# 21cmfast/21cmFAST

Hardware: AMD Instinct MI355X
Metric: IonizeBox cells/sec (512^3 HII_DIM, 40 filter radii) (higher is better)
Workload: dtype f32; 1 GPU; ComputeIonizedBox single-z, HII_DIM=512, 40 filter steps, G=2 (delta tophat + n_ion exp-MFP), first snapshot, device-resident inputs; hii_dim=512, n_radii=40, filtered_grids=2, parallelism=single GPU, fft=native

## Files before the change

### 21cmfast_amd/csrc/hip/c21hip.h

```cpp
#ifndef C21HIP_H
#define C21HIP_H

#include <stddef.h>

#include "ws_slots.h"

#ifdef __cplusplus
extern "C" {
#endif

int c21hip_device_count(void);
int c21hip_current_device(void);
int c21hip_use_device(int device);
int c21hip_is_device_ptr(const void *p);
void *c21hip_ws(int slot, size_t bytes);
__attribute__((visibility("hidden"))) const void *c21_stage_in(int slot, const void *p, size_t bytes, void *stream, int *status);
void *c21hip_ws_peek(int slot, size_t *bytes);
int c21hip_ws_adopt(int slot, void *ptr, size_t bytes);
void *c21hip_raw_alloc(size_t bytes);
void *c21hip_vmm_chunk(size_t phys_bytes, size_t map_bytes, void **va_out);
void c21hip_vmm_chunk_free(void *chunk);
int c21hip_ws_adopt_vmm(int slot, void *chunk, size_t bytes);
void c21hip_raw_free(void *p);
size_t c21hip_free_bytes(void);
// ... 146 lines not shown
int c21hip_split_fold_multi(const float *hi_split, float *const lo_split[4], const int ops[4], int n_out, int nx,
                            int ny, int nz, int f, double box_len, double box_len_z, float tophat_R, void *stream);
int c21hip_lpt2_source(const float *const diag[3], const float *const off[3], float *out, size_t n,
                       float norm, void *stream);
int c21hip_copy_filter_split(const float *src_split, float *dst_split, int nx, int ny, int nz,
                             double box_len, double box_len_z, int filter_type, float R,
                             float R_param, int apply, void *stream);
int c21hip_split_z_c2r(const float *split_work, float *real_out, long out_zstride, int nx, int ny,
                       int nz, void *stream);
int c21hip_split_z_ionise_stars(const float *delta_work, const float *stars_work,
                                unsigned char *first_cross, double *partials, double *sum_out,
                                int nx, int ny, int nz, int r_index, double rhocrit_omb,
                                double ion_eff, int mass_dep_zeta, double f_limit, void *stream);
int c21hip_z_ionise_partials(int nx, int ny, int nz);
int c21hip_batched_means(const double *partials, long stride, int n_partials, int first, int step,
                         int count, double ntot, int mass_dep_zeta, double f_limit, double *sums,
                         double *means, void *stream);
int c21hip_split_z_ionise_stars_xe(const float *delta_work, const float *stars_work,
                                   const float *xe_work, unsigned char *first_cross,
                                   double *partials, double *sum_out, int nx, int ny, int nz,
                                   int r_index, double rhocrit_omb, double ion_eff,
                                   int mass_dep_zeta, double f_limit, void *stream);
int c21hip_z_ionise_xe_supported(int nx, int ny, int nz);
int c21hip_split_filter_xy_shared(const float *src, float *work, int filter_type, int nx, int ny,
                                  int nz, double box_len, double box_len_z, float R, int apply,
                                  int table_slot, void *stream);
int c21hip_bench_pass(int kind, int n, int filter_a, int filter_b, float R, float R_param_b,
                      double box_len, int reps, void *stream, float *ms_out);
int c21hip_reduce_sum(const double *partials, int n, double *out, void *stream);
int c21hip_reduce_op(const double *partials, int n, int op, double *stage, double *out,
                     void *stream);

int c21hip_pack_clip(const float *dense, float *padded, int nx, int ny, int nz, double factor,
                     double lo, double hi, void *stream);
int c21hip_unpack_scale(const float *padded, float *dense, int nx, int ny, int nz, float scale,
                        void *stream);
int c21hip_divide_inplace(float *buf, size_t n, float divisor, void *stream);
int c21hip_divide_inplace_f64(float *buf, size_t n, double divisor, void *stream);
int c21hip_fill(float *buf, size_t n, float value, void *stream);
int c21hip_add_scalar(float *buf, size_t n, float value, void *stream);
int c21hip_widen(const float *in, double *out, size_t n, void *stream);

int c21hip_copy_filter(const float *src_c, float *dst_c, int nx, int ny, int nz, double box_len,
                       double box_len_z, int filter_type, float R, float R_param, int apply,
                       void *stream);
int c21hip_copy_filter_star(const float *src_c, float *dst_c, int nx, int ny, int nz,
// ... 377 lines not shown
```

### 21cmfast_amd/csrc/hip/fft_native.hip

```cpp
#include <hip/hip_runtime.h>

#include <cmath>
#include <map>
#include <mutex>
#include <vector>

#include "c21hip.h"
#include "fcoll_device.h"
#include "ms_window.h"
#include "c21cm_abi.h"
#include "c21cm_grid.h"

#ifndef C21X_XPAIR_THREADS
#define C21X_XPAIR_THREADS 512
#endif
#ifndef C21X_FUSE512
#define C21X_FUSE512 1
#endif
#ifndef C21X_FUSE1024
#define C21X_FUSE1024 1
#endif
#ifndef C21X_F512_MERGE
#define C21X_F512_MERGE 1
#endif
// ... 1536 lines not shown
        } else {
            const float2 A = tile[k * ZROW + li], B = tile[(H - k) * ZROW + li];
            const float2 E = make_float2(0.5f * (A.x + B.x), 0.5f * (A.y - B.y));
            const float2 D = make_float2(0.5f * (A.x - B.x), 0.5f * (A.y + B.y));
            const float2 wD = cmul(D, twN[k]);
            tile[k * ZROW + li] = make_float2(E.x + wD.y, E.y - wD.x);
            tile[(H - k) * ZROW + li] = make_float2(E.x - wD.y, -E.y - wD.x);
        }
    }
    __syncthreads();
#pragma unroll
    for (int u = 0; u < NIN; u++) {
        const int f = threadIdx.x + kBlock * u;
        const int li = f / H, k = f % H;
        a.main[(l0 + li) * H + k] = tile[k * ZROW + li];
    }
}

struct ZFusedArgs {
    const float2 *d_main, *d_nyq;
    const float2 *s_main, *s_nyq;
    const float2 *x_main, *x_nyq;
    unsigned char *first_cross;
    double *partials;
    double rhocrit_omb, ion_eff, f_limit;
    int mass_dep_zeta, r_index;
    int ny, lb;
    int store_all;
    int reverse;
    int rc;
    const float *nrec;
    double rec0;
    int x_is_nrec;
    const float2 *n_main, *n_nyq;
    float *g12;
};

template <int NZ>
__global__ void __launch_bounds__(kBlock)
z_c2r_ionise_kernel(ZFusedArgs a, const float2 *__restrict__ twH_global,
                    const float2 *__restrict__ twN_global) {
    constexpr int H = NZ / 2, LZ = LZ_FUSED, ZROW = LZ + 1;
    constexpr int NOUT = ZGeom<NZ, LZ>::NOUT;
    extern __shared__ float4 lds_raw[];
    float2 *tile = reinterpret_cast<float2 *>(lds_raw);
    float2 *twH = tile + H * ZROW;
// ... 267 lines not shown

template <int NZ, int EPI = 0>
int launch_z_c2r(const ZPassArgs &a, long nlines, hipStream_t stream) {
    constexpr int H = NZ / 2;
    const float2 *twH = twiddles(H);
    const float2 *twN = twiddles(NZ);
    if (!twH || !twN) return C21CM_MEMORY_ALLOC_ERROR;
    const size_t lds = sizeof(float2) * ((size_t)H * (LZ_PLAIN + 1) + H + H / 2 + 1);
    static bool attr_done = false;
    if (!attr_done) {
        (void)hipFuncSetAttribute((const void *)z_c2r_kernel<NZ, EPI>,
                                  hipFuncAttributeMaxDynamicSharedMemorySize, (int)lds);
        attr_done = true;
    }
    hipLaunchKernelGGL((z_c2r_kernel<NZ, EPI>), dim3((unsigned)(nlines / LZ_PLAIN)), dim3(kBlock),
                       lds, stream, a, twH, twN);
    LAUNCH_CHECK();
    return 0;
}

constexpr int ZW_LINES = 16;
constexpr int zw_lines(int P) { return kBlock / P; }

template <int A, bool TS, int P = 16, bool RC = false>
__global__ void
#if C21X_ZW_OCC
__launch_bounds__(kBlock, (A == 16 && !TS) ? C21X_ZW_OCC : 1)
#else
__launch_bounds__((A == 16 && P == 16) ? C21X_ZW_BLOCK : kBlock, (TS && RC && A == 16 && P == 16) ? C21X_ZW_TSRC_OCC : 1)
#endif
zw_ionise_kernel(ZFusedArgs a, const float2 *__restrict__ twH_global,
                 const float2 *__restrict__ twN_global) {
    constexpr int ZBLK = (A == 16 && P == 16) ? C21X_ZW_BLOCK : kBlock;
    constexpr int H = P * A, NZ = 2 * H, ZWL = ZBLK / P;
    constexpr int LINE_LDS = A * (P + 1) + 4;
    static_assert(LINE_LDS % 2 == 0, "16-byte aligned line regions (mask rows)");
    __shared__ __attribute__((aligned(16))) float2 lines[ZWL * LINE_LDS];
    __shared__ float2 twH[H], twN[H];
    __shared__ double red[ZBLK / 64];
    for (int t = threadIdx.x; t < H; t += ZBLK) {
        twH[t] = twH_global[t];
        twN[t] = twN_global[t];
    }
    const int lane = threadIdx.x & 63, wave = threadIdx.x >> 6;
    const int g = lane / P, b = lane % P;
    const int lw = wave * (64 / P) + g;
    const unsigned blk = a.reverse ? gridDim.x - 1 - blockIdx.x : blockIdx.x;
    const long line = (long)blk * ZWL + lw;
    float2 *L = lines + lw * LINE_LDS;
    const float2 *dm = a.d_main + line * H, *sm = a.s_main + line * H;
    constexpr bool EARLY = (A == 16) && !C21X_ZW_LATE;
    float2 xd[A], xs[A];
#pragma unroll
    for (int q = 0; q < A; q++) xd[q] = dm[P * q + b];
    if (EARLY) {
#pragma unroll
        for (int q = 0; q < A; q++) xs[q] = sm[P * q + b];
    }
    const long lline = logical_line(line, a.ny, a.lb);
    const float dh = a.d_nyq[lline].x, sh = a.s_nyq[lline].x;
    unsigned char *mrow = a.first_cross + lline * NZ;
    constexpr bool MASK16 = EARLY && (C21X_ZW_MASK16 || (TS && RC && C21X_ZW_TSRC_LEAN));
    constexpr int MV = MASK16 ? A / 8 : 1;
    uint4 mreg[MV];
    uchar2 old[(EARLY && !MASK16) ? A : 1];
    if constexpr (MASK16) {
#pragma unroll
        for (int v = 0; v < MV; v++) mreg[v] = reinterpret_cast<const uint4 *>(mrow)[b * MV + v];
    } else if (EARLY) {
#pragma unroll
        for (int q = 0; q < A; q++)
            old[q] = reinterpret_cast<const uchar2 *>(mrow)[(b + P * (q / P)) + A * (q % P)];
    }
    constexpr bool STASH = TS && RC && A == 16 && P == 16 && C21X_ZW_TSRC_LEAN;
    constexpr int NRH = (RC && A == 16 && !STASH) ? A / 2 : 1;
    float2 nr_lo[NRH], nr_hi[NRH];
    __shared__ __attribute__((aligned(16))) float nstash[STASH ? ZWL * NZ : 4];
    uint4 nreg[STASH ? NZ / (4 * P) : 1];
    if constexpr (STASH) {
#pragma unroll
        for (int v = 0; v < NZ / (4 * P); v++) nreg[v] = make_uint4(0u, 0u, 0u, 0u);
        if (a.nrec) {
#pragma unroll
            for (int v = 0; v < NZ / (4 * P); v++)
                nreg[v] = reinterpret_cast<const uint4 *>(a.nrec + lline * NZ)[v * P + b];
        }
    } else if constexpr (RC && A == 16) {
        if (a.nrec) {
#pragma unroll
            for (int q = 0; q < NRH; q++)
                nr_lo[q] = reinterpret_cast<const float2 *>(a.nrec + lline * NZ)[(b + P * (q / P)) + A * (q % P)];
        }
// ... 39 lines not shown
        wave_fence();
        wave_c2r<A, P>(xx, xh, L, twH, twN, b);
    }

    if constexpr (RC && A == 16 && !STASH) {
        if (a.nrec) {
#pragma unroll
            for (int q = 0; q < NRH; q++) {
                const int qq = q + NRH;
                nr_hi[q] = reinterpret_cast<const float2 *>(a.nrec + lline * NZ)[(b + P * (qq / P)) + A * (qq % P)];
            }
        }
    }
    if constexpr (MASK16) {
        wave_fence();
#pragma unroll
        for (int v = 0; v < MV; v++) reinterpret_cast<uint4 *>(L)[b * MV + v] = mreg[v];
        wave_fence();
    }
    const double floor_lhs = a.f_limit * a.ion_eff;
    const bool floor_ionises = !TS && a.mass_dep_zeta && (floor_lhs > 1.);
    const float dmin = (float)(-1. + 1e-7);
    double acc = 0.;
#pragma unroll
    for (int q = 0; q < A; q++) {
        const int j = (b + P * (q / P)) + A * (q % P);
        const float s0 = fmaxf(xs[q].x, 0.f), s1 = fmaxf(xs[q].y, 0.f);
        acc += (double)s0;
        acc += (double)s1;
        double D0 = a.rhocrit_omb * (1. + (double)fmaxf(xd[q].x, dmin));
        double D1 = a.rhocrit_omb * (1. + (double)fmaxf(xd[q].y, dmin));
        bool f0 = false, f1 = false;
        if constexpr (TS) {
            const double n0 = 1. - (double)fminf(fmaxf(xx[q].x, 0.f), 0.999f);
            const double n1 = 1. - (double)fminf(fmaxf(xx[q].y, 0.f), 0.999f);
            f0 = a.mass_dep_zeta && floor_lhs > n0;
            f1 = a.mass_dep_zeta && floor_lhs > n1;
            D0 *= n0;
            D1 *= n1;
        }
        double opd0 = 1., opd1 = 1.;
        if constexpr (RC) {
            opd0 = 1. + (double)fmaxf(xd[q].x, dmin);
            opd1 = 1. + (double)fmaxf(xd[q].y, dmin);
            double r0 = a.rec0, r1 = a.rec0;
            if (a.nrec || (STASH && a.n_main)) {
                const float2 nr = STASH ? reinterpret_cast<const float2 *>(nstash + lw * NZ)[j]
                                  : (A == 16) ? (q < NRH ? nr_lo[(A == 16 && !STASH && q < NRH) ? q : 0]
                                                         : nr_hi[(A == 16 && !STASH && q >= NRH) ? q - NRH : 0])
                                              : reinterpret_cast<const float2 *>(a.nrec + lline * NZ)[j];
                r0 = (double)nr.x, r1 = (double)nr.y;
            }
            double n0 = 1., n1 = 1.;
            if constexpr (TS) {
                if (a.x_is_nrec) {
                    r0 = (double)fmaxf(xx[q].x, 0.f);
                    r1 = (double)fmaxf(xx[q].y, 0.f);
                } else {
                    n0 = 1. - (double)fminf(fmaxf(xx[q].x, 0.f), 0.999f);
                    n1 = 1. - (double)fminf(fmaxf(xx[q].y, 0.f), 0.999f);
                }
            }
            D0 = a.rhocrit_omb * ((opd0 + r0) * n0);
            D1 = a.rhocrit_omb * ((opd1 + r1) * n1);
            f0 = a.mass_dep_zeta && floor_lhs * opd0 > (opd0 + r0) * n0;
            f1 = a.mass_dep_zeta && floor_lhs * opd1 > (opd1 + r1) * n1;
        }
        const bool i0 = (!RC && floor_ionises) || f0 || ((double)s0 * a.ion_eff > D0);
        const bool i1 = (!RC && floor_ionises) || f1 || ((double)s1 * a.ion_eff > D1);
        uchar2 m = MASK16 ? reinterpret_cast<const uchar2 *>(L)[j]
                          : (EARLY ? old[(EARLY && !MASK16) ? q : 0] : reinterpret_cast<const uchar2 *>(mrow)[j]);
        const bool n0 = i0 && m.x == 0, n1 = i1 && m.y == 0;
        if (n0) m.x = (unsigned char)a.r_index;
        if (n1) m.y = (unsigned char)a.r_index;
        if constexpr (MASK16) {
            if (n0 || n1) reinterpret_cast<uchar2 *>(L)[j] = m;
        } else if (n0 || n1 || a.store_all)
            reinterpret_cast<uchar2 *>(mrow)[j] = m;
        if constexpr (RC) {
            float *grow = a.g12 + lline * NZ + 2 * j;
            if (n0 && a.rc != 2) grow[0] = fmaxf(xd[q].x, dmin);
            if (n1 && a.rc != 2) grow[1] = fmaxf(xd[q].y, dmin);
        }
#if C21X_ZW_TSRC_FENCE
        if constexpr (TS && RC) __builtin_amdgcn_sched_barrier(0);
#endif
    }
    if constexpr (MASK16) {
        wave_fence();
#pragma unroll
        for (int v = 0; v < MV; v++) {
            const uint4 n = reinterpret_cast<const uint4 *>(L)[b * MV + v], o = mreg[v];
            if (a.store_all || n.x != o.x || n.y != o.y || n.z != o.z || n.w != o.w)
                reinterpret_cast<uint4 *>(mrow)[b * MV + v] = n;
        }
    }
#pragma unroll
    for (int off = 32; off > 0; off >>= 1) acc += __shfl_down(acc, off, 64);
    if (lane == 0) red[wave] = acc;
    __syncthreads();
    if (threadIdx.x == 0) {
        double sum = 0.;
#pragma unroll
        for (int w = 0; w < ZBLK / 64; w++) sum += red[w];
        a.partials[blk] = sum;
    }
}

template <int A, int EPI, int P = 16>
__global__ void __launch_bounds__(kBlock)
zw_c2r_kernel(ZPassArgs a, const float2 *__restrict__ twH_global,
              const float2 *__restrict__ twN_global) {
    constexpr int H = P * A, NZ = 2 * H, ZWL = zw_lines(P);
    constexpr int LINE_LDS = A * (P + 1) + 4;
    static_assert(LINE_LDS % 2 == 0, "16-byte aligned line regions (EPI 7)");
    __shared__ __attribute__((aligned(16))) float2 lines[ZWL * LINE_LDS];
    __shared__ float2 twH[H], twN[H];
    for (int t = threadIdx.x; t < H; t += kBlock) {
        twH[t] = twH_global[t];
// ... 597 lines not shown

template <int NZ>
int launch_z_fused(const ZFusedArgs &a, long nlines, hipStream_t stream) {
    constexpr int H = NZ / 2;
    const float2 *twH = twiddles(H);
    const float2 *twN = twiddles(NZ);
    if (!twH || !twN) return C21CM_MEMORY_ALLOC_ERROR;
    const size_t lds = sizeof(float2) * ((size_t)H * (LZ_FUSED + 1) + H + H / 2 + 1);
    static bool attr_done = false;
    if (!attr_done) {
        (void)hipFuncSetAttribute((const void *)z_c2r_ionise_kernel<NZ>,
                                  hipFuncAttributeMaxDynamicSharedMemorySize, (int)lds);
        attr_done = true;
    }
    hipLaunchKernelGGL((z_c2r_ionise_kernel<NZ>), dim3((unsigned)(nlines / LZ_FUSED)), dim3(kBlock), lds,
                       stream, a, twH, twN);
    LAUNCH_CHECK();
    return 0;
}

int dispatch_z_fused(int nz, const ZFusedArgs &a, long nlines, hipStream_t stream, int *n_partials) {
    KTimeScope kt(2, stream);
    *n_partials = (int)(nlines / LZ_FUSED);
    if (a.rc && (zw3_selected(nz, nlines) || !zw_lines_of(nz, nlines))) {
        c21hip_set_error("fused pass Z with recombinations needs the 16-lane wave kernel (z-lines of 256 / 512 points)");
        return C21CM_VALUE_ERROR;
    }
    if (zw3_selected(nz, nlines)) {
        const float2 *twH = twiddles(nz / 2);
        const float2 *twN = twiddles(nz);
        if (!twH || !twN) return C21CM_MEMORY_ALLOC_ERROR;
        *n_partials = (int)(nlines / (kBlock / 64));
        const dim3 grid((unsigned)(nlines / (kBlock / 64)));
        if (a.x_main)
            hipLaunchKernelGGL(zw3_ionise_kernel<true>, grid, dim3(kBlock), 0, stream, a, twH, twN);
        else
            hipLaunchKernelGGL(zw3_ionise_kernel<false>, grid, dim3(kBlock), 0, stream, a, twH, twN);
        LAUNCH_CHECK();
        return 0;
    }
    if (int zwl = zw_lines_of(nz, nlines)) {
        const float2 *twH = twiddles(nz / 2);
        const float2 *twN = twiddles(nz);
        if (!twH || !twN) return C21CM_MEMORY_ALLOC_ERROR;
        const int zblk = (nz == 512) ? C21X_ZW_BLOCK : kBlock;
        if (nz == 512) zwl = zblk / 16;
// ... 8 lines not shown
                hipLaunchKernelGGL((zw_ionise_kernel<16, true, 8, true>), grid, dim3(zblk), 0, stream, a, twH, twN);
            else if (nz == 512)
                hipLaunchKernelGGL((zw_ionise_kernel<16, true, 16, true>), grid, dim3(zblk), 0, stream, a, twH, twN);
            else {
                c21hip_set_error("fused pass Z with recombinations and an x_e grid: 256- / 512-point z-lines only");
                return C21CM_VALUE_ERROR;
            }
        } else if (a.rc) {
            if (nz == 256)
                ZW_FUSED_RC(16, 8);
            else if (nz == 512)
                ZW_FUSED_RC(16, 16);
            else
                ZW_FUSED_RC(32, 16);
        } else if (a.x_main) {
            if (nz == 256)
                ZW_FUSED(16, true, 8);
            else if (nz == 512)
                ZW_FUSED(16, true, 16);
            else
                ZW_FUSED(32, true, 16);
        } else if (nz == 256)
            ZW_FUSED(16, false, 8);
        else if (nz == 512)
            ZW_FUSED(16, false, 16);
        else
            ZW_FUSED(32, false, 16);
#undef ZW_FUSED
#undef ZW_FUSED_RC
        LAUNCH_CHECK();
        return 0;
    }
    if (a.x_main) {
        c21hip_set_error("fused pass Z with an x_e grid needs 256-, 512- or 1024-point z-lines");
        return C21CM_VALUE_ERROR;
    }
    switch (nz) {
        case 64: return launch_z_fused<64>(a, nlines, stream);
        case 128: return launch_z_fused<128>(a, nlines, stream);
        case 192: return launch_z_fused<192>(a, nlines, stream);
        case 256: return launch_z_fused<256>(a, nlines, stream);
        case 384: return launch_z_fused<384>(a, nlines, stream);
        case 512: return launch_z_fused<512>(a, nlines, stream);
        case 768: return launch_z_fused<768>(a, nlines, stream);
        case 1024: return launch_z_fused<1024>(a, nlines, stream);
        case 1536: return launch_z_fused<1536>(a, nlines, stream);
// ... 1194 lines not shown
    return c21hip_reduce_sum(partials, (int)(nlines / LZ_PLAIN), sum_out, stream);
}

extern "C" int c21hip_split_filter_c2r(const float *split_src, float *split_work, float *real_out,
                                       long out_zstride, int nx, int ny, int nz, double box_len,
                                       double box_len_z, int filter_type, float R, float R_param,
                                       int apply, void *stream) {
    int st = c21hip_split_filter_xy(split_src, split_work, nx, ny, nz, box_len, box_len_z,
                                    filter_type, R, R_param, apply, stream);
    if (st) return st;
    return c21hip_split_z_c2r(split_work, real_out, out_zstride, nx, ny, nz, stream);
}

extern "C" int c21hip_split_z_ionise_stars(const float *delta_work, const float *stars_work,
                                           unsigned char *first_cross, double *partials,
                                           double *sum_out, int nx, int ny, int nz, int r_index,
                                           double rhocrit_omb, double ion_eff, int mass_dep_zeta,
                                           double f_limit, void *stream) {
    return c21hip_split_z_ionise_stars_xe(delta_work, stars_work, NULL, first_cross, partials,
                                          sum_out, nx, ny, nz, r_index, rhocrit_omb, ion_eff,
                                          mass_dep_zeta, f_limit, stream);
}

extern "C" int c21hip_split_z_ionise_stars_xe(const float *delta_work, const float *stars_work,
                                              const float *xe_work, unsigned char *first_cross,
                                              double *partials, double *sum_out, int nx, int ny,
                                              int nz, int r_index, double rhocrit_omb,
                                              double ion_eff, int mass_dep_zeta, double f_limit,
                                              void *stream) {
    const long nlines = (long)nx * ny;
    ZFusedArgs a{};
    a.ny = ny;
    a.lb = split_xb_log2(nx);
    a.d_main = reinterpret_cast<const float2 *>(delta_work);
    a.d_nyq = a.d_main + nlines * (nz / 2);
    a.s_main = reinterpret_cast<const float2 *>(stars_work);
    a.s_nyq = a.s_main + nlines * (nz / 2);
    if (xe_work) {
        a.x_main = reinterpret_cast<const float2 *>(xe_work);
        a.x_nyq = a.x_main + nlines * (nz / 2);
    }
    a.first_cross = first_cross;
    a.partials = partials;
    a.rhocrit_omb = rhocrit_omb;
    a.ion_eff = ion_eff;
    a.f_limit = f_limit;
    a.mass_dep_zeta = mass_dep_zeta;
    a.r_index = r_index;
    static const int store_all = [] {
        const char *e = getenv("C21CM_MASK_STORE_ALL");
        return (e && e[0] == '1') ? 1 : 0;
    }();
    a.store_all = store_all;
    static const int reverse = [] {
        const char *e = getenv("C21CM_ZREV");
        return (e && e[0] == '0') ? 0 : 1;
    }();
    a.reverse = reverse;
    int n_partials = 0;
    int st = dispatch_z_fused(nz, a, nlines, (hipStream_t)stream, &n_partials);
    if (st) return st;
    if (!sum_out) return 0;
    return c21hip_reduce_sum(partials, n_partials, sum_out, stream);
}

extern "C" int c21hip_split_z_ionise_recomb_xe(const float *delta_work, const float *stars_work,
                                               const float *xe_work, const float *nrec, double rec0,
                                               float *g12, unsigned char *first_cross, double *partials,
                                               int nx, int ny, int nz, int r_index, double rhocrit_omb,
                                               double ion_eff, int mass_dep_zeta, double f_limit,
                                               void *stream);
extern "C" int c21hip_split_z_ionise_recomb(const float *delta_work, const float *stars_work,
                                            const float *nrec, double rec0, float *g12,
                                            unsigned char *first_cross,
                                            double *partials, int nx, int ny, int nz, int r_index,
                                            double rhocrit_omb, double ion_eff, int mass_dep_zeta,
                                            double f_limit, void *stream) {
    return c21hip_split_z_ionise_recomb_xe(delta_work, stars_work, nullptr, nrec, rec0, g12, first_cross,
                                           partials, nx, ny, nz, r_index, rhocrit_omb, ion_eff,
                                           mass_dep_zeta, f_limit, stream);
}
extern "C" int c21hip_split_z_ionise_recomb_xe(const float *delta_work, const float *stars_work,
                                               const float *xe_work, const float *nrec, double rec0,
                                               float *g12, unsigned char *first_cross, double *partials,
                                               int nx, int ny, int nz, int r_index, double rhocrit_omb,
                                               double ion_eff, int mass_dep_zeta, double f_limit,
// ... 387 lines not shown
        }
    }
    hipEvent_t e0, e1;
    if (hipEventCreate(&e0) != hipSuccess || hipEventCreate(&e1) != hipSuccess)
        return C21CM_IO_ERROR;
    for (int r = -2; r < reps && !st; r++) {
        if (r == 0) (void)hipEventRecord(e0, stream);
        if (kind == 0 || kind == 7)
            st = filter_xy(src, work, 2, n, n, n, box_len, box_len, ft, R, rp, 1, stream_, 2);
        else if (kind == 8)
            st = filter_xy_pair(a, real, pair2[0], filter_a, 0.f, b, real2, pair2[1], filter_b,
                                R_param_b, n, n, n, box_len, box_len, R, 0.9f * R, 0, 1, 2,
                                stream_);
        else if (kind == 1)
            st = filter_xy(src, work, 2, n, n, n, box_len, box_len, ft, R, rp, 1, stream_, 4);
        else if (kind == 4)
            st = filter_xy(src, work, 2, n, n, n, box_len, box_len, ft, R, rp, 1, stream_, 1);
        else if (kind == 6)
            st = filter_xy_pair(a, real, pair2[0], filter_a, 0.f, b, real2, pair2[1], filter_b,
                                R_param_b, n, n, n, box_len, box_len, R, 0.9f * R, 0, 1, 2,
                                stream_);
        else if (kind == 5)
            st = filter_xy(src, work, 2, n, n, n, box_len, box_len, ft, R, rp, 0, stream_, 2);
        else if (kind == 2)
            st = c21hip_split_z_ionise_stars(a, b, mask, partials, partials + nlines / 4 + 40,
                                             n, n, n, 5, 6.2e9, 1.0, 1, 1e-9, stream);
        else {
            ZPassArgs z{};
            z.ny = n;
            z.lb = split_xb_log2(n);
            z.main = reinterpret_cast<const float2 *>(a);
            z.nyq = z.main + nlines * H;
            z.out = real;
            z.out_zstride = n + 2;
            z.out_scale = 1.0f;
            st = dispatch_z_c2r(n, z, nlines, stream);
        }
    }
    (void)hipEventRecord(e1, stream);
    (void)hipEventSynchronize(e1);
    float ms = 0.f;
    (void)hipEventElapsedTime(&ms, e0, e1);
    (void)hipEventDestroy(e0);
    (void)hipEventDestroy(e1);
    *ms_out = ms / (float)reps;
    if (kind == 7 || kind == 8) c21hip_wev_release();
// ... 14 lines not shown
```

### 21cmfast_amd/csrc/hip/ionize_kernels.hip

```cpp
#include <hip/hip_runtime.h>

#include <cmath>
#include <cstdint>

#include "c21hip.h"
#include "c21cm_abi.h"
#include "c21cm_grid.h"
#include "fcoll_device.h"

namespace {
constexpr int kBlock = 256;
constexpr int kMaxBlocks = 256 * 8;
constexpr double kTiny = 1e-30;
constexpr double kMinDensityLowLimit = 9e-8;

inline int grid_for(size_t work_items) {
    size_t b = (work_items + kBlock - 1) / kBlock;
    if (b > (size_t)kMaxBlocks) b = kMaxBlocks;
    if (b < 1) b = 1;
    return (int)b;
}

#define LAUNCH_CHECK()                                                                  \
    do {                                                                                \
// ... 1032 lines not shown
                acc_x += (double)x;
                if (!a.minimize_memory) {
                    if (zr > 0.f && (double)x < kTiny) {
                        T = fully_ionized_T(zr, stored_z, dens, pow_Tre, pow_z);
                        if (T < T_neutral) T = T_neutral;
                    }
                    if (!isfinite(T)) bad = 1;
                }
                xo.v[e] = x;
                zo.v[e] = zr;
                To.v[e] = T;
            }
            xo.store(xH, i);
            zo.store(z_reion, i);
            if (!a.minimize_memory) To.store(Tk, i);
        }
    }
    if (bad) atomicOr(flag, 1);
    block_sum_to(acc_s, partials_stars + chunk0);
    __syncthreads();
    block_sum_to(acc_x, partials_xh + chunk0);
}

__global__ void __launch_bounds__(kBlock)
apply_first_cross_kernel(const unsigned char *__restrict__ fc,
                         const float *__restrict__ prev_z_reion, int first_snapshot, float z_now,
                         float *__restrict__ xH, float *__restrict__ z_reion, size_t ntot) {
    for (size_t i = (size_t)blockIdx.x * kBlock + threadIdx.x; i < ntot;
         i += (size_t)gridDim.x * kBlock) {
        if (fc[i]) {
            const float pz = first_snapshot ? -1.f : prev_z_reion[i];
            z_reion[i] = (pz < 0.f) ? z_now : pz;
            xH[i] = 0.f;
        }
    }
}

__global__ void __launch_bounds__(kBlock)
apply_first_cross_recomb_kernel(const unsigned char *__restrict__ fc, const float *__restrict__ R_dev,
                                const float *__restrict__ prev_z_reion, int first_snapshot,
                                float z_now, float *__restrict__ xH, float *__restrict__ z_reion,
                                float *__restrict__ mfp, size_t ntot) {
    for (size_t i = (size_t)blockIdx.x * kBlock + threadIdx.x; i < ntot;
         i += (size_t)gridDim.x * kBlock) {
        const unsigned char r = fc[i];
        if (r) {
// ... 700 lines not shown
                                           const float *prev_z_reion, float *xH, float *z_reion,
                                           float *kinetic_temperature, double *partials, double *sum_xh_out,
                                           int *flag_out, const float *xe_dense,
                                           const float *kinetic_temp_neutral, void *stream) {
    const int st = c21hip_final_sweep_eulerian_range(a, stored_redshift, first_cross, nion_dense, mean_dev,
                                                     density, prev_z_reion, xH, z_reion, kinetic_temperature,
                                                     partials, flag_out, xe_dense, kinetic_temp_neutral, 0, -1,
                                                     stream);
    if (st) return st;
    return c21hip_final_sweep_reduce(a, 1, partials, nullptr, sum_xh_out, stream);
}

extern "C" int c21hip_brightness_temp(const float *density, const float *xH, const float *Ts,
                                      float *bt, float *tau, size_t n, float const_factor,
                                      float T_rad, double redshift, int use_ts, double *partials,
                                      double *sum_out, void *stream) {
    const int blocks = grid_for(n);
    hipLaunchKernelGGL(brightness_kernel, dim3(blocks), dim3(kBlock), 0, (hipStream_t)stream,
                       density, xH, Ts, bt, tau, n, const_factor, T_rad, redshift, use_ts,
                       partials);
    LAUNCH_CHECK();
    hipLaunchKernelGGL(finish_reduce_kernel, dim3(1), dim3(kBlock), 0, (hipStream_t)stream,
                       partials, blocks, 0, sum_out);
    LAUNCH_CHECK();
    return 0;
}

extern "C" int c21hip_apply_first_cross(const unsigned char *first_cross,
                                        const float *prev_z_reion, int first_snapshot,
                                        double redshift, float *xH, float *z_reion, size_t ntot,
                                        void *stream) {
    hipLaunchKernelGGL(apply_first_cross_kernel, dim3(grid_for(ntot)), dim3(kBlock), 0,
                       (hipStream_t)stream, first_cross, prev_z_reion, first_snapshot,
                       (float)redshift, xH, z_reion, ntot);
    LAUNCH_CHECK();
    return 0;
}

extern "C" int c21hip_apply_first_cross_recomb(const unsigned char *first_cross, const float *R_dev,
                                               const float *prev_z_reion, int first_snapshot,
                                               double redshift, float *xH, float *z_reion,
                                               float *mfp, size_t ntot, void *stream) {
    hipLaunchKernelGGL(apply_first_cross_recomb_kernel, dim3(grid_for(ntot)), dim3(kBlock), 0,
                       (hipStream_t)stream, first_cross, R_dev, prev_z_reion, first_snapshot,
                       (float)redshift, xH, z_reion, mfp, ntot);
    LAUNCH_CHECK();
// ... 553 lines not shown
```

### 21cmfast_amd/csrc/hip/ws_slots.h

```cpp
#ifndef C21_WS_SLOTS_H
#define C21_WS_SLOTS_H

enum c21_ws_slot {
    WS_DELTA_UNF,
    WS_DELTA_FIL,
    WS_STARS_UNF,
    WS_STARS_FIL,
    WS_XE_UNF,
    WS_XE_FIL,
    WS_DENSITY,
    WS_NION,
    WS_XE_DENSE,
    WS_TNEUTRAL,
    WS_PREV_ZRE,
    WS_XH,
    WS_ZRE,
    WS_TK,
    WS_NION_DENSE,
    WS_SCALARS,
    WS_TABLE,
    WS_FIRST_CROSS,
    WS_DELTA_WORK,
    WS_STARS_WORK,
    WS_XE_WORK,
    WS_PT_LOW = WS_XE_WORK,
    WS_PARTIALS,
    WS_PT_HIGH = WS_PARTIALS,

    WS_PT_SAVED,
    WS_PT_RESAMPLED,
    WS_HB_ACC0 = WS_PT_RESAMPLED,
    WS_PT_IN0,
    WS_PT_IN_LAST = WS_PT_IN0 + 6,
    WS_HB_IN0 = WS_PT_IN0,
    WS_HB_IN_LAST = WS_PT_IN_LAST,
    WS_PT_OUT0,
    WS_PT_OUT_LAST = WS_PT_OUT0 + 3,
    WS_HB_OUT0 = WS_PT_OUT0,
    WS_HB_OUT_LAST = WS_PT_OUT0 + 2,
    WS_HB_ACC1 = WS_PT_OUT_LAST,

    WS_BT_DENS,
    WS_BT_XH,
    WS_BT_TS,
// ... 239 lines not shown
```

### 21cmfast_amd/csrc/host/ionize_driver.c

```c
#include <math.h>
#include <stdio.h>
#include <stdlib.h>
#include <string.h>

#include "../hip/c21hip.h"
#include "c21cm_grid.h"

#define MAX_COPYBACK 12
typedef struct {
    void *host[MAX_COPYBACK];
    void *dev[MAX_COPYBACK];
    size_t bytes[MAX_COPYBACK];
    int n;
} copyback_list;

#define SC_SUMS 0
#define SC_MEANS (SC_SUMS + C21CM_MAX_RADII)
#define SC_MINMAX (SC_MEANS + C21CM_MAX_RADII)
#define SC_XHSUM (SC_MINMAX + 4)
#define SC_FLAG (SC_XHSUM + 1)
#define SC_G12SUM (SC_FLAG + 1)
#define SC_SUMS_M (SC_G12SUM + 1)
#define SC_MEANS_M (SC_SUMS_M + C21CM_MAX_RADII)
#define SC_MINMAX_M (SC_MEANS_M + C21CM_MAX_RADII)
// ... 186 lines not shown
    int wev;
    int fused_rc;
    int eul_pend, eul_pend_buf;
    unsigned char *eul_pend_mask;
    float *nion_dense2;
    int band_off;
    int band_used;
    int band_next;
    int band_pend;
    int band_h1, band_h2, band_hn;
    unsigned char *band_mask;
    const unsigned char *r0_mask;
    int r0_slab, r0_cb, r0_ce;
    int band_mf;
    int band_skip;
    short band_hist[C21CM_MAX_RADII][3];
    float *band_xe_pend;
    const float *cur_xe;
    int x3_on, x3_nrec;
    float *x3_unf, *x3_work, *x3_work2;
    int x4_on;
    float *x4_unf, *x4_work, *x4_work2;
    const float *cur_x4;
    float *sfr_work2;
    double rec0;
    int finalised;
    float *eul_xe[2];
    int wev_pair, pairx_R;
    float *pairx_buf;
    int sphere;
    int mini, lag_mini;
    float *pd_unf, *pd_work, *pd_fil, *mta_unf, *mta_work, *mta_fil, *mtm_unf, *mtm_work, *mtm_fil;
    const float *prev_density, *mta_dense, *mtm_dense, *hist_a, *hist_m;
    float *mini_tables, *nion_all, *mini_all;
    int eul_mask;
    copyback_list cb;
    size_t cb_cell0, cb_ncell;
} ion_ctx;

static int r0_direct(void);

static int g_loop_flags;
int c21cm_ionize_last_loop_flags(void) { return g_loop_flags; }

static int ctx_setup(ion_ctx *c, const c21cm_ionize_spec *s, const PerturbedField *pf,
                     const IonizedBox *prev, const TsBox *ts, const HaloBox *halos,
// ... 386 lines not shown
        st = c21hip_d2d(c->nion_dense, c->nion_dense2, c->ntot * sizeof(float), c->stream);
    return st;
}

static int flush_deferred(ion_ctx *c) {
    {
        const int st_e = eul_flush_pending(c, 1);
        if (st_e) return st_e;
    }
    if (!c->def_partials || c->def_count == 0) return 0;
    const c21cm_ionize_spec *s = c->s;
    int st = c21hip_batched_means(c->def_partials, c->def_stride, (int)c->def_stride, c->def_first,
                                  c->def_count > 1 ? c->def_step : 1, c->def_count,
                                  (double)c->ntot, s->mass_dep_zeta, s->f_limit_acg,
                                  c->scalars + SC_SUMS, c->scalars + SC_MEANS, c->stream);
    c->def_count = 0;
    return st;
}

static int z_ionise_radius(ion_ctx *c, int R_ct, const float *dwork, const float *swork,
                           const float *xwork, unsigned char *first_cross) {
    int status = 0;
    const c21cm_ionize_spec *s = c->s;
    if (c->fused_rc) {
        double *part = c->def_partials ? c->def_partials + (long)R_ct * c->def_stride : c->partials;
        if (c->def_partials) {
            if (c->def_count == 0)
                c->def_first = R_ct;
            else if (c->def_count == 1)
                c->def_step = c->def_first - R_ct;
            else if (R_ct != c->def_first - c->def_count * c->def_step)
                TRY(flush_deferred(c));
            if (c->def_count == 0) c->def_first = R_ct;
            c->def_count++;
        }
        if (c->x4_on)
            TRY(c21hip_split_z_ionise_recomb_xe_nrec(dwork, swork, c->cur_xe, c->cur_x4, c->G12, first_cross,
                                                     part, c->nx, c->ny, c->nz, R_ct, s->rhocrit_omb,
                                                     s->ion_eff_factor, s->mass_dep_zeta, s->f_limit_acg,
                                                     c->stream));
        else if (c->x3_nrec)
            TRY(c21hip_split_z_ionise_recomb_nrec(dwork, swork, c->cur_xe, c->G12, first_cross, part, c->nx,
                                                  c->ny, c->nz, R_ct, s->rhocrit_omb, s->ion_eff_factor,
                                                  s->mass_dep_zeta, s->f_limit_acg, c->stream));
        else
        TRY(c21hip_split_z_ionise_recomb_xe(dwork, swork, s->use_ts_fluct ? c->cur_xe : NULL,
                                            c->inhomo ? c->prev_nrec : NULL, c->rec0, c->G12, first_cross,
                                            part, c->nx, c->ny, c->nz, R_ct, s->rhocrit_omb,
                                            s->ion_eff_factor, s->mass_dep_zeta, s->f_limit_acg, c->stream));
        TRY(c21hip_split_z_sfr_gamma12(xwork, first_cross, c->G12, c->nx, c->ny, c->nz, R_ct,
                                       s->R[R_ct] * s->gamma_prefactor, c->stream));
        if (!c->def_partials) {
            double *sum_dev = c->scalars + SC_SUMS + R_ct;
            TRY(c21hip_reduce_sum(part, c21hip_z_ionise_partials(c->nx, c->ny, c->nz), sum_dev, c->stream));
            TRY(c21hip_finish_mean(sum_dev, (double)c->ntot, s->mass_dep_zeta, s->f_limit_acg,
                                   c->scalars + SC_MEANS + R_ct, c->stream));
        }
        goto done;
    }
    if (c->def_partials) {
        if (c->def_count == 0)
            c->def_first = R_ct;
        else if (c->def_count == 1)
            c->def_step = c->def_first - R_ct;
        else if (R_ct != c->def_first - c->def_count * c->def_step)
            TRY(flush_deferred(c));
        if (c->def_count == 0) c->def_first = R_ct;
        c->def_count++;
        TRY(c21hip_split_z_ionise_stars_xe(dwork, swork, xwork, first_cross,
                                           c->def_partials + (long)R_ct * c->def_stride, NULL,
                                           c->nx, c->ny, c->nz, R_ct, s->rhocrit_omb,
                                           s->ion_eff_factor, s->mass_dep_zeta, s->f_limit_acg,
                                           c->stream));
        goto done;
    }
    {
        double *sum_dev = c->scalars + SC_SUMS + R_ct;
        TRY(c21hip_split_z_ionise_stars_xe(dwork, swork, xwork, first_cross, c->partials, sum_dev,
                                           c->nx, c->ny, c->nz, R_ct, s->rhocrit_omb,
                                           s->ion_eff_factor, s->mass_dep_zeta, s->f_limit_acg,
                                           c->stream));
        TRY(c21hip_finish_mean(sum_dev, (double)c->ntot, s->mass_dep_zeta, s->f_limit_acg,
                               c->scalars + SC_MEANS + R_ct, c->stream));
    }
done:
    return status;
}

static int fused_step(ion_ctx *c, int R_a, int R_b, unsigned char *first_cross, int next_a,
                      int next_b) {
    int status = 0;
    const c21cm_ionize_spec *s = c->s;
    const int set = c->tab_seq & 1;
    const int buf_a = 2 * set, buf_b = 2 * set + 1;
    tab_init();
    const int tab_async = !c->wev && g_tab.enabled && c->ntot >= ((size_t)1 << 26);
    if (tab_async) {
        if (c->tab_seq == 0) {
            TRY(c21hip_event_record(g_tab.ev_sync, c->stream));
            TRY(c21hip_stream_wait_event(g_tab.aux, g_tab.ev_sync));
// ... 1157 lines not shown
                                 c->stream));
    if (c->sphere) TRY(paint_spheres(c, mask));
    if (s->r_lowest == 0) TRY(one_radius(c, 0, NULL, -1));
done:
    return status;
}

static int finish_first_cross_recomb(ion_ctx *c, const unsigned char *mask) {
    int status = 0;
    const c21cm_ionize_spec *s = c->s;
    float Rf[C21CM_MAX_RADII];
    for (int r = 0; r < C21CM_MAX_RADII; r++) Rf[r] = r < s->n_radii ? (float)s->R[r] : 0.f;
    float *R_dev = (float *)c21hip_ws(WS_R_DEV, sizeof(Rf));
    if (!R_dev) return C21CM_MEMORY_ALLOC_ERROR;
    TRY(c21hip_h2d(R_dev, Rf, sizeof(Rf), c->stream));
    TRY(c21hip_sync(c->stream));
    TRY(c21hip_apply_first_cross_recomb(mask, R_dev, c->prev_zre, s->first_snapshot, s->redshift, c->xH,
                                        c->zre, c->mfp, c->ntot, c->stream));
    TRY(one_radius(c, 0, NULL, -1));
done:
    return status;
}

int c21cm_ionize_grids(const c21cm_ionize_spec *spec, const PerturbedField *perturbed_field,
                       const IonizedBox *previous_ionize_box, const TsBox *spin_temp,
                       const HaloBox *halos, IonizedBox *box, c21cm_ionize_report *report,
                       void *stream) {
    int status = validate_spec(spec, perturbed_field, halos, spin_temp, box);
    if (status) return status;
    ion_ctx c;
    phase_clock clk = {{NULL}, 0, 0};
    unsigned char *mask = NULL;
    g_spectra.valid = 0;
    TRY(ctx_setup(&c, spec, perturbed_field, previous_ionize_box, spin_temp, halos, box, 1, 1, stream));
    TRY(clock_start(&clk, 4, stream));
    TRY(init_output_grids(&c, previous_ionize_box));
    TRY(preloop(&c));
    TRY(clock_mark(&clk, stream));
    if (c.fused || c.eul_mask || c.sphere) {
        mask = (unsigned char *)c21hip_ws(WS_FIRST_CROSS, c.ntot);
        if (!mask) {
            status = C21CM_MEMORY_ALLOC_ERROR;
            goto done;
        }
        TRY(c21hip_memset(mask, 0, c.ntot, stream));
    }
    TRY(native_wev_prepare(&c));
    if (mask) {
        TRY(radii_ladder(&c, spec->n_radii - 1, 1, mask, spec->r_lowest == 0 ? 0 : -1));
        TRY(flush_deferred(&c));
        TRY(c.fused_rc ? finish_first_cross_recomb(&c, mask) : finish_first_cross(&c, mask, 0));
    } else {
        for (int R_ct = spec->n_radii - 1; R_ct >= spec->r_lowest; R_ct--)
            TRY(one_radius(&c, R_ct, NULL, -1));
        TRY(flush_deferred(&c));
    }
    c21hip_wev_release();
    TRY(clock_mark(&clk, stream));
    TRY(postloop(&c, box, report));
    TRY(clock_mark(&clk, stream));
    if (report) {
        report->ms_preloop = clock_ms(&clk, 0);
        report->ms_rloop = clock_ms(&clk, 1);
        report->ms_postloop = clock_ms(&clk, 2);
    }
done:
    c21hip_wev_release();
    clock_free(&clk);
    return status;
}

static int no_mini_shards(void) {
// ... 549 lines not shown
```

Baseline: 3.272 billion cells/s.

## Record per-radius ionisation crossings as bit planes and resolve first-cross afterward

In the fused two-grid z-pass on 512-point lines, the kernel no longer reads and writes the per-cell first-cross byte mask for every radius. Each thread instead packs its ionisation flags into one 32-bit word per radius plane. A separate resolve kernel runs once after the radius ladder, walks the planes from largest to smallest radius, and writes the first-crossing radius index into the byte mask. This replaces a byte-mask read-modify-write on every step with a compact bit write, at the cost of (n_radii-1)*ntot/8 bytes of extra workspace and one extra pass over all planes at the end.

```diff
diff --git a/21cmfast_amd/csrc/hip/c21hip.h b/21cmfast_amd/csrc/hip/c21hip.h
--- a/21cmfast_amd/csrc/hip/c21hip.h
+++ b/21cmfast_amd/csrc/hip/c21hip.h
@@ -192,6 +192,13 @@
                                    int r_index, double rhocrit_omb, double ion_eff,
                                    int mass_dep_zeta, double f_limit, void *stream);
 int c21hip_z_ionise_xe_supported(int nx, int ny, int nz);
+int c21hip_z_cross_bits_supported(int nx, int ny, int nz);
+int c21hip_split_z_ionise_stars_bits(const float *delta_work, const float *stars_work,
+                                     unsigned *cross_plane, double *partials, double *sum_out, int nx,
+                                     int ny, int nz, int r_index, double rhocrit_omb, double ion_eff,
+                                     int mass_dep_zeta, double f_limit, void *stream);
+int c21hip_resolve_crossings(const unsigned *bits, int r_hi, int r_lo, unsigned char *first_cross,
+                             size_t nlines, void *stream);
 int c21hip_split_filter_xy_shared(const float *src, float *work, int filter_type, int nx, int ny,
                                   int nz, double box_len, double box_len_z, float R, int apply,
                                   int table_slot, void *stream);
diff --git a/21cmfast_amd/csrc/hip/fft_native.hip b/21cmfast_amd/csrc/hip/fft_native.hip
--- a/21cmfast_amd/csrc/hip/fft_native.hip
+++ b/21cmfast_amd/csrc/hip/fft_native.hip
@@ -1582,6 +1582,7 @@
     const float2 *s_main, *s_nyq;
     const float2 *x_main, *x_nyq;
     unsigned char *first_cross;
+    unsigned *cross_bits;
     double *partials;
     double rhocrit_omb, ion_eff, f_limit;
     int mass_dep_zeta, r_index;
@@ -1895,7 +1896,7 @@
 constexpr int ZW_LINES = 16;
 constexpr int zw_lines(int P) { return kBlock / P; }
 
-template <int A, bool TS, int P = 16, bool RC = false>
+template <int A, bool TS, int P = 16, bool RC = false, bool CB = false>
 __global__ void
 #if C21X_ZW_OCC
 __launch_bounds__(kBlock, (A == 16 && !TS) ? C21X_ZW_OCC : 1)
@@ -1923,6 +1924,7 @@
     float2 *L = lines + lw * LINE_LDS;
     const float2 *dm = a.d_main + line * H, *sm = a.s_main + line * H;
     constexpr bool EARLY = (A == 16) && !C21X_ZW_LATE;
+    static_assert(!CB || (A == 16 && P == 16 && !TS && !RC), "crossing bits: the two-grid kernel on 512-point lines");
     float2 xd[A], xs[A];
 #pragma unroll
     for (int q = 0; q < A; q++) xd[q] = dm[P * q + b];
@@ -1932,15 +1934,16 @@
     }
     const long lline = logical_line(line, a.ny, a.lb);
     const float dh = a.d_nyq[lline].x, sh = a.s_nyq[lline].x;
-    unsigned char *mrow = a.first_cross + lline * NZ;
-    constexpr bool MASK16 = EARLY && (C21X_ZW_MASK16 || (TS && RC && C21X_ZW_TSRC_LEAN));
+    unsigned char *mrow = nullptr;
+    if constexpr (!CB) mrow = a.first_cross + lline * NZ;
+    constexpr bool MASK16 = !CB && EARLY && (C21X_ZW_MASK16 || (TS && RC && C21X_ZW_TSRC_LEAN));
     constexpr int MV = MASK16 ? A / 8 : 1;
     uint4 mreg[MV];
     uchar2 old[(EARLY && !MASK16) ? A : 1];
     if constexpr (MASK16) {
 #pragma unroll
         for (int v = 0; v < MV; v++) mreg[v] = reinterpret_cast<const uint4 *>(mrow)[b * MV + v];
-    } else if (EARLY) {
+    } else if (EARLY && !CB) {
 #pragma unroll
         for (int q = 0; q < A; q++)
             old[q] = reinterpret_cast<const uchar2 *>(mrow)[(b + P * (q / P)) + A * (q % P)];
@@ -2026,6 +2029,7 @@
     const bool floor_ionises = !TS && a.mass_dep_zeta && (floor_lhs > 1.);
     const float dmin = (float)(-1. + 1e-7);
     double acc = 0.;
+    unsigned cb = 0u;
 #pragma unroll
     for (int q = 0; q < A; q++) {
         const int j = (b + P * (q / P)) + A * (q % P);
@@ -2072,6 +2076,10 @@
         }
         const bool i0 = (!RC && floor_ionises) || f0 || ((double)s0 * a.ion_eff > D0);
         const bool i1 = (!RC && floor_ionises) || f1 || ((double)s1 * a.ion_eff > D1);
+        if constexpr (CB) {
+            cb |= (i0 ? (1u << q) : 0u) | (i1 ? (0x10000u << q) : 0u);
+            continue;
+        }
         uchar2 m = MASK16 ? reinterpret_cast<const uchar2 *>(L)[j]
                           : (EARLY ? old[(EARLY && !MASK16) ? q : 0] : reinterpret_cast<const uchar2 *>(mrow)[j]);
         const bool n0 = i0 && m.x == 0, n1 = i1 && m.y == 0;
@@ -2099,6 +2107,7 @@
                 reinterpret_cast<uint4 *>(mrow)[b * MV + v] = n;
         }
     }
+    if constexpr (CB) a.cross_bits[lline * (NZ / 32) + b] = cb;
 #pragma unroll
     for (int off = 32; off > 0; off >>= 1) acc += __shfl_down(acc, off, 64);
     if (lane == 0) red[wave] = acc;
@@ -2742,6 +2751,10 @@
 int dispatch_z_fused(int nz, const ZFusedArgs &a, long nlines, hipStream_t stream, int *n_partials) {
     KTimeScope kt(2, stream);
     *n_partials = (int)(nlines / LZ_FUSED);
+    if (a.cross_bits && !(nz == 512 && zw_lines_of(nz, nlines) && !a.rc && !a.x_main)) {
+        c21hip_set_error("fused pass Z: crossing bits need the two-grid wave kernel on 512-point z-lines");
+        return C21CM_VALUE_ERROR;
+    }
     if (a.rc && (zw3_selected(nz, nlines) || !zw_lines_of(nz, nlines))) {
         c21hip_set_error("fused pass Z with recombinations needs the 16-lane wave kernel (z-lines of 256 / 512 points)");
         return C21CM_VALUE_ERROR;
@@ -2796,6 +2809,8 @@
                 ZW_FUSED(32, true, 16);
         } else if (nz == 256)
             ZW_FUSED(16, false, 8);
+        else if (nz == 512 && a.cross_bits)
+            hipLaunchKernelGGL((zw_ionise_kernel<16, false, 16, false, true>), grid, dim3(zblk), 0, stream, a, twH, twN);
         else if (nz == 512)
             ZW_FUSED(16, false, 16);
         else
@@ -4036,12 +4051,10 @@
                                           mass_dep_zeta, f_limit, stream);
 }
 
-extern "C" int c21hip_split_z_ionise_stars_xe(const float *delta_work, const float *stars_work,
-                                              const float *xe_work, unsigned char *first_cross,
-                                              double *partials, double *sum_out, int nx, int ny,
-                                              int nz, int r_index, double rhocrit_omb,
-                                              double ion_eff, int mass_dep_zeta, double f_limit,
-                                              void *stream) {
+static int z_ionise_stars(const float *delta_work, const float *stars_work, const float *xe_work,
+                          unsigned char *first_cross, unsigned *cross_bits, double *partials,
+                          double *sum_out, int nx, int ny, int nz, int r_index, double rhocrit_omb,
+                          double ion_eff, int mass_dep_zeta, double f_limit, void *stream) {
     const long nlines = (long)nx * ny;
     ZFusedArgs a{};
     a.ny = ny;
@@ -4055,6 +4068,7 @@
         a.x_nyq = a.x_main + nlines * (nz / 2);
     }
     a.first_cross = first_cross;
+    a.cross_bits = cross_bits;
     a.partials = partials;
     a.rhocrit_omb = rhocrit_omb;
     a.ion_eff = ion_eff;
@@ -4076,6 +4090,37 @@
     if (st) return st;
     if (!sum_out) return 0;
     return c21hip_reduce_sum(partials, n_partials, sum_out, stream);
+}
+
+extern "C" int c21hip_split_z_ionise_stars_xe(const float *delta_work, const float *stars_work,
+                                              const float *xe_work, unsigned char *first_cross,
+                                              double *partials, double *sum_out, int nx, int ny,
+                                              int nz, int r_index, double rhocrit_omb,
+                                              double ion_eff, int mass_dep_zeta, double f_limit,
+                                              void *stream) {
+    return z_ionise_stars(delta_work, stars_work, xe_work, first_cross, nullptr, partials, sum_out, nx,
+                          ny, nz, r_index, rhocrit_omb, ion_eff, mass_dep_zeta, f_limit, stream);
+}
+
+extern "C" int c21hip_z_cross_bits_supported(int nx, int ny, int nz) {
+    static const int on = [] {
+        const char *e = getenv("C21CM_CROSS_BITS");
+        return (e && e[0] == '0') ? 0 : 1;
+    }();
+    return on && nz == 512 && zw_lines_of(nz, (long)nx * ny) != 0;
+}
+
+extern "C" int c21hip_split_z_ionise_stars_bits(const float *delta_work, const float *stars_work,
+                                                unsigned *cross_plane, double *partials,
+                                                double *sum_out, int nx, int ny, int nz, int r_index,
+                                                double rhocrit_omb, double ion_eff,
+                                                int mass_dep_zeta, double f_limit, void *stream) {
+    if (!cross_plane || !c21hip_z_cross_bits_supported(nx, ny, nz)) {
+        c21hip_set_error("fused pass Z: crossing bits are not available for this grid");
+        return C21CM_VALUE_ERROR;
+    }
+    return z_ionise_stars(delta_work, stars_work, nullptr, nullptr, cross_plane, partials, sum_out, nx,
+                          ny, nz, r_index, rhocrit_omb, ion_eff, mass_dep_zeta, f_limit, stream);
 }
 
 extern "C" int c21hip_split_z_ionise_recomb_xe(const float *delta_work, const float *stars_work,
@@ -4509,6 +4554,10 @@
                                 stream_);
         else if (kind == 5)
             st = filter_xy(src, work, 2, n, n, n, box_len, box_len, ft, R, rp, 0, stream_, 2);
+        else if (kind == 2 && c21hip_z_cross_bits_supported(n, n, n))
+            st = c21hip_split_z_ionise_stars_bits(a, b, reinterpret_cast<unsigned *>(mask), partials,
+                                                  partials + nlines / 4 + 40, n, n, n, 5, 6.2e9, 1.0, 1,
+                                                  1e-9, stream);
         else if (kind == 2)
             st = c21hip_split_z_ionise_stars(a, b, mask, partials, partials + nlines / 4 + 40,
                                              n, n, n, 5, 6.2e9, 1.0, 1, 1e-9, stream);
diff --git a/21cmfast_amd/csrc/hip/ionize_kernels.hip b/21cmfast_amd/csrc/hip/ionize_kernels.hip
--- a/21cmfast_amd/csrc/hip/ionize_kernels.hip
+++ b/21cmfast_amd/csrc/hip/ionize_kernels.hip
@@ -1078,6 +1078,47 @@
     block_sum_to(acc_x, partials_xh + chunk0);
 }
 
+template <int NS>
+__global__ void __launch_bounds__(kBlock)
+resolve_crossings_kernel(const unsigned *__restrict__ bits, size_t plane_words, int r_hi, int r_lo,
+                         unsigned char *__restrict__ first_cross, size_t nquads) {
+    const size_t t = (size_t)blockIdx.x * kBlock + threadIdx.x;
+    if (t >= nquads) return;
+    unsigned seen[4] = {0u, 0u, 0u, 0u}, sl[NS][4];
+#pragma unroll
+    for (int s = 0; s < NS; s++)
+#pragma unroll
+        for (int i = 0; i < 4; i++) sl[s][i] = 0u;
+#pragma unroll 4
+    for (int r = r_hi; r >= r_lo; r--) {
+        const uint4 w = reinterpret_cast<const uint4 *>(bits + (size_t)(r - 1) * plane_words)[t];
+        const unsigned wv[4] = {w.x, w.y, w.z, w.w};
+#pragma unroll
+        for (int i = 0; i < 4; i++) {
+            const unsigned fresh = wv[i] & ~seen[i];
+            seen[i] |= wv[i];
+#pragma unroll
+            for (int s = 0; s < NS; s++)
+                if ((r >> s) & 1) sl[s][i] |= fresh;
+        }
+    }
+    unsigned char *row = first_cross + (t >> 2) * 512 + 8 * (t & 3);
+#pragma unroll
+    for (int q = 0; q < 16; q++) {
+        unsigned v[4];
+#pragma unroll
+        for (int i = 0; i < 4; i++) {
+            v[i] = 0u;
+#pragma unroll
+            for (int s = 0; s < NS; s++) v[i] |= ((sl[s][i] >> q) & 0x00010001u) << s;
+        }
+        uint2 o;
+        o.x = (v[0] & 0xffu) | ((v[0] >> 16) << 8) | ((v[1] & 0xffu) << 16) | ((v[1] >> 16) << 24);
+        o.y = (v[2] & 0xffu) | ((v[2] >> 16) << 8) | ((v[3] & 0xffu) << 16) | ((v[3] >> 16) << 24);
+        *reinterpret_cast<uint2 *>(row + 32 * q) = o;
+    }
+}
+
 __global__ void __launch_bounds__(kBlock)
 apply_first_cross_kernel(const unsigned char *__restrict__ fc,
                          const float *__restrict__ prev_z_reion, int first_snapshot, float z_now,
@@ -1824,6 +1865,24 @@
     LAUNCH_CHECK();
     hipLaunchKernelGGL(finish_reduce_kernel, dim3(1), dim3(kBlock), 0, (hipStream_t)stream,
                        partials, blocks, 0, sum_out);
+    LAUNCH_CHECK();
+    return 0;
+}
+
+extern "C" int c21hip_resolve_crossings(const unsigned *bits, int r_hi, int r_lo,
+                                        unsigned char *first_cross, size_t nlines, void *stream) {
+    if (r_lo < 1 || r_hi > 255 || !nlines) {
+        c21hip_set_error("resolve_crossings: radius indices 1..255 and at least one line");
+        return C21CM_VALUE_ERROR;
+    }
+    const size_t nquads = nlines * 4;
+    const dim3 grid((unsigned)((nquads + kBlock - 1) / kBlock));
+    if (r_hi < 64)
+        hipLaunchKernelGGL(resolve_crossings_kernel<6>, grid, dim3(kBlock), 0, (hipStream_t)stream, bits,
+                           nlines * 16, r_hi, r_lo, first_cross, nquads);
+    else
+        hipLaunchKernelGGL(resolve_crossings_kernel<8>, grid, dim3(kBlock), 0, (hipStream_t)stream, bits,
+                           nlines * 16, r_hi, r_lo, first_cross, nquads);
     LAUNCH_CHECK();
     return 0;
 }
diff --git a/21cmfast_amd/csrc/hip/ws_slots.h b/21cmfast_amd/csrc/hip/ws_slots.h
--- a/21cmfast_amd/csrc/hip/ws_slots.h
+++ b/21cmfast_amd/csrc/hip/ws_slots.h
@@ -20,6 +20,7 @@
     WS_SCALARS,
     WS_TABLE,
     WS_FIRST_CROSS,
+    WS_CROSS_BITS,
     WS_DELTA_WORK,
     WS_STARS_WORK,
     WS_XE_WORK,
diff --git a/21cmfast_amd/csrc/host/ionize_driver.c b/21cmfast_amd/csrc/host/ionize_driver.c
--- a/21cmfast_amd/csrc/host/ionize_driver.c
+++ b/21cmfast_amd/csrc/host/ionize_driver.c
@@ -232,6 +232,7 @@
     int x4_on;
     float *x4_unf, *x4_work, *x4_work2;
     const float *cur_x4;
+    unsigned *cross_bits;
     float *sfr_work2;
     double rec0;
     int finalised;
@@ -664,6 +665,7 @@
                            const float *xwork, unsigned char *first_cross) {
     int status = 0;
     const c21cm_ionize_spec *s = c->s;
+    unsigned *plane = c->cross_bits ? c->cross_bits + (size_t)(R_ct - 1) * (c->ntot / 32) : NULL;
     if (c->fused_rc) {
         double *part = c->def_partials ? c->def_partials + (long)R_ct * c->def_stride : c->partials;
         if (c->def_partials) {
@@ -709,6 +711,13 @@
             TRY(flush_deferred(c));
         if (c->def_count == 0) c->def_first = R_ct;
         c->def_count++;
+        if (plane)
+            TRY(c21hip_split_z_ionise_stars_bits(dwork, swork, plane,
+                                                 c->def_partials + (long)R_ct * c->def_stride, NULL,
+                                                 c->nx, c->ny, c->nz, R_ct, s->rhocrit_omb,
+                                                 s->ion_eff_factor, s->mass_dep_zeta, s->f_limit_acg,
+                                                 c->stream));
+        else
         TRY(c21hip_split_z_ionise_stars_xe(dwork, swork, xwork, first_cross,
                                            c->def_partials + (long)R_ct * c->def_stride, NULL,
                                            c->nx, c->ny, c->nz, R_ct, s->rhocrit_omb,
@@ -718,6 +727,11 @@
     }
     {
         double *sum_dev = c->scalars + SC_SUMS + R_ct;
+        if (plane)
+            TRY(c21hip_split_z_ionise_stars_bits(dwork, swork, plane, c->partials, sum_dev, c->nx, c->ny,
+                                                 c->nz, R_ct, s->rhocrit_omb, s->ion_eff_factor,
+                                                 s->mass_dep_zeta, s->f_limit_acg, c->stream));
+        else
         TRY(c21hip_split_z_ionise_stars_xe(dwork, swork, xwork, first_cross, c->partials, sum_dev,
                                            c->nx, c->ny, c->nz, R_ct, s->rhocrit_omb,
                                            s->ion_eff_factor, s->mass_dep_zeta, s->f_limit_acg,
@@ -1921,6 +1935,15 @@
     return status;
 }
 
+static void cross_bits_begin(ion_ctx *c) {
+    const c21cm_ionize_spec *s = c->s;
+    c->cross_bits = NULL;
+    if (!c->fused || c->fused_rc || s->use_ts_fluct || c->sphere || s->n_radii < 2 ||
+        !c21hip_z_cross_bits_supported(c->nx, c->ny, c->nz))
+        return;
+    c->cross_bits = (unsigned *)c21hip_ws(WS_CROSS_BITS, (size_t)(s->n_radii - 1) * (c->ntot / 8));
+}
+
 int c21cm_ionize_grids(const c21cm_ionize_spec *spec, const PerturbedField *perturbed_field,
                        const IonizedBox *previous_ionize_box, const TsBox *spin_temp,
                        const HaloBox *halos, IonizedBox *box, c21cm_ionize_report *report,
@@ -1942,11 +1965,18 @@
             status = C21CM_MEMORY_ALLOC_ERROR;
             goto done;
         }
-        TRY(c21hip_memset(mask, 0, c.ntot, stream));
+        cross_bits_begin(&c);
+        if (!c.cross_bits)
+            TRY(c21hip_memset(mask, 0, c.ntot, stream));
     }
     TRY(native_wev_prepare(&c));
     if (mask) {
         TRY(radii_ladder(&c, spec->n_radii - 1, 1, mask, spec->r_lowest == 0 ? 0 : -1));
+        if (c.cross_bits) {
+            TRY(c21hip_resolve_crossings(c.cross_bits, spec->n_radii - 1, spec->r_lowest > 1 ? spec->r_lowest : 1,
+                                         mask, (size_t)c.nx * c.ny, stream));
+            c.cross_bits = NULL;
+        }
         TRY(flush_deferred(&c));
         TRY(c.fused_rc ? finish_first_cross_recomb(&c, mask) : finish_first_cross(&c, mask, 0));
     } else {
```

After: 3.454 billion cells/s (median of 6 runs). +5.6%, better.
